# MuLabPKU/HD-PiSSA

Hardware: AMD Instinct MI355X
Metric: train tokens/sec (node) on the HD-PiSSA hot path, llama2-7b r16 (adapter probe fwd/bwd + Adam + dW aggregate + merge); dW merge+gather ms/step (higher is better)
Workload: dtype f32; 1 GPU; llama2-7b; model=llama2-7b, global_batch=16, seq_len=512, padding=per micro-batch to its longest sample (hp:190-201), micro_batches_per_rank=8, r_per_gpu=16, modules=224, exchange=gather, parallelism=dp1 (HD-PiSSA slices), x_layout=shared per projection group (q/k/v, gate/up)

## Files before the change

### hd-pissa_amd/csrc/hdp_probe.hip

```cpp
#include <chrono>
#include <cstdlib>
#include <cstring>
#include <mutex>
#include <vector>

#include "hdp_probe_int.h"

namespace hdp {

constexpr int kMaxGroup = 1024;
constexpr int kMaxSplit = 16;
constexpr int kP1Waves = 8;

static int p1_cols() {
  static const int v = [] { const char* e = getenv("HDP_P1_COLS"); return e ? atoi(e) : 128; }();
  return v;
}
static int p1_u() {
  static const int v = [] { const char* e = getenv("HDP_P1_U"); return e ? atoi(e) : 1; }();
  return v;
}
constexpr int kTC = 128;
constexpr int kNW = 256;

// ... 414 lines not shown
        const int j = 16 * b + 4 * g + reg;
        if (j >= r) continue;
        float* p = d.g + (int64_t)j * N + col;
        const f32x4 v{sc * acc2[b][0][reg], sc * acc2[b][1][reg], sc * acc2[b][2][reg], sc * acc2[b][3][reg]};
        if (vec) {
          gst4(p, d.acc ? gld4(p) + v : v);
        } else {
#pragma unroll
          for (int q = 0; q < 4; ++q)
            if (col + q < N) gst1(p + q, d.acc ? gld1(p + q) + v[q] : v[q]);
        }
      }
  } else {
    const bool v4 = (d.ldb & 3) == 0 && (reinterpret_cast<uintptr_t>(d.g) & 15) == 0;
#pragma unroll
    for (int b = 0; b < RB; ++b)
#pragma unroll
      for (int q = 0; q < 4; ++q) {
        if (col + q >= N) continue;
        const int j0 = 16 * b + 4 * g;
        float* p = d.g + (col + q) * d.ldb + j0;
        const f32x4 v = sc * acc2[b][q];
        if (v4 && j0 + 3 < r) {
          gst4(p, d.acc ? gld4(p) + v : v);
        } else {
#pragma unroll
          for (int reg = 0; reg < 4; ++reg)
            if (j0 + reg < r) gst1(p + reg, d.acc ? gld1(p + reg) + v[reg] : v[reg]);
        }
      }
  }
}

__device__ __forceinline__ void sw_store_g_fuse(const SweepDesc& d, const f32x4 (&acc2)[kSwMaxBlk][4], int64_t col,
                                                int g, bool vec) {
#pragma clang fp contract(off)
  const int64_t N = d.N;
  if (!d.part_t) {
#pragma unroll
    for (int b = 0; b < kSwMaxBlk; ++b) {
      if (b >= d.nb) break;
      const float sc = d.sc[b];
      const int acc = d.accb[b];
#pragma unroll
      for (int reg = 0; reg < 4; ++reg) {
        const int j = 4 * g + reg;
        if (j >= d.rbr[b]) continue;
        float* p = d.gb[b] + (int64_t)j * N + col;
        const f32x4 v{sc * acc2[b][0][reg], sc * acc2[b][1][reg], sc * acc2[b][2][reg], sc * acc2[b][3][reg]};
        if (vec) {
          gst4(p, acc ? gld4(p) + v : v);
        } else {
#pragma unroll
          for (int q = 0; q < 4; ++q)
            if (col + q < N) gst1(p + q, acc ? gld1(p + q) + v[q] : v[q]);
        }
      }
    }
  } else {
    const float sc = d.scale;
    const int r = d.r;
    const bool v4 = (d.ldb & 3) == 0 && (reinterpret_cast<uintptr_t>(d.g) & 15) == 0;
#pragma unroll
    for (int b = 0; b < kSwMaxBlk; ++b) {
      if (b >= d.nb) break;
#pragma unroll
      for (int q = 0; q < 4; ++q) {
        if (col + q >= N) continue;
        const int j0 = 16 * b + 4 * g;
        float* p = d.g + (col + q) * d.ldb + j0;
        const f32x4 v = sc * acc2[b][q];
        if (v4 && j0 + 3 < r) {
          gst4(p, d.acc ? gld4(p) + v : v);
        } else {
#pragma unroll
          for (int reg = 0; reg < 4; ++reg)
            if (j0 + reg < r) gst1(p + reg, d.acc ? gld1(p + reg) + v[reg] : v[reg]);
        }
      }
    }
  }
}

struct SweepArgs {
  int n, G;
  int spin;
  int64_t U;
  int* err;
  int* errd;
  const SweepDesc* d;
  const int* wst;
  const int* bnd;
};

template <int DT, int RB, int MODE, bool VEC, int OCC, bool FUSE, bool K32>
__device__ __forceinline__ void sweep_segment(const SweepDesc& d, int ct, int s0, int n, int64_t i0, int piece,
                                              const SweepArgs& sa, float* tile, float* red, int* flags, int wave,
                                              int lane) {
  constexpr bool PROJ = (MODE & kSwProj) != 0, OUTER = (MODE & kSwOuter) != 0;
  constexpr int rp = 16 * RB, r4 = rp / 4, ES = DT == HDP_F32 ? 4 : 2;
  const int li = lane & 15, g = lane >> 4;
  const int64_t T = d.T, N = d.N;
  const int64_t c = (int64_t)ct * kSwC + 64 * wave;
  const int64_t col = c + 4 * li;
  const int64_t colc = VEC ? (col < N ? col : N - 4) : col;
  const char* Zb = reinterpret_cast<const char*>(d.Z);

  constexpr bool SPLIT_F = DT == HDP_BF16 && MODE == kSwProj;
  constexpr bool X6 = K32 && DT == HDP_F32;
  constexpr bool K32P = K32 && MODE == kSwProj, K32O = K32 && MODE == kSwOuter;
  constexpr bool DL = K32P && DT == HDP_BF16 && !X6 && VEC;
  const int64_t cdl0 = c + 8 * g < N ? c + 8 * g : N - 8, cdl1 = c + 32 + 8 * g < N ? c + 32 + 8 * g : N - 8;
  f32x4 f[K32P ? 1 : 4][RB];
  bf16x4 fs[K32P ? 1 : 4][RB][3];
  bf16x8 fs8[K32P ? 2 : 1][RB][3];
  if constexpr (K32P) {
#pragma unroll
    for (int ch = 0; ch < 2; ++ch)
#pragma unroll
      for (int b = 0; b < RB; ++b) {
        const int j = 16 * b + li;
        const int64_t k = c + 32 * ch + 8 * g;
        float v[8];
#pragma unroll
        for (int e = 0; e < 8; ++e) v[e] = 0.f;
        const float* Fp = nullptr;
        int rows = d.r;
        if constexpr (FUSE) {
          Fp = b < d.nb ? d.Fb[b] : nullptr;
          rows = b < d.nb ? d.rbr[b] : 0;
        }
        const bool ok = FUSE ? (Fp != nullptr && li < rows) : (j < d.r);
        if (ok) {
          if (FUSE) Fp += (int64_t)li * N;
          if ((FUSE || d.f_rk) && N % 4 == 0 && k + 7 < N) {
            const float* P = FUSE ? Fp : d.F + (int64_t)j * N;
            const f32x4 a = gld4(P + k), bq = gld4(P + k + 4);
#pragma unroll
            for (int e = 0; e < 4; ++e) {
              v[e] = a[e];
              v[4 + e] = bq[e];
            }
          } else {
#pragma unroll
            for (int e = 0; e < 8; ++e)
              if (k + e < N)
                v[e] = FUSE ? gld1(Fp + k + e)
                            : d.f_rk ? gld1(d.F + (int64_t)j * N + k + e) : gld1(d.F + (k + e) * d.r + j);
          }
        }
        split8(v, fs8[ch][b][0], fs8[ch][b][1], fs8[ch][b][2]);
#pragma unroll
        for (int t = 0; t < 3; ++t) asm volatile("" : "+v"(fs8[ch][b][t]));
      }
  }
  if constexpr (PROJ && !K32P) {
#pragma unroll
    for (int s = 0; s < 4; ++s)
#pragma unroll
      for (int b = 0; b < RB; ++b) {
        const int j = 16 * b + li;
        const int64_t k = c + 16 * s + 4 * g;
        f32x4 v{0.f, 0.f, 0.f, 0.f};
        if constexpr (FUSE) {
          if (b < d.nb && li < d.rbr[b]) {
            const float* Fp = d.Fb[b] + (int64_t)li * N;
// ... 414 lines not shown
        load(z0, y0);
        if (k + 1 < nfull) compute(z1, y1, s0 + k + 1, i0 + k + 1, false);
      }
    }
  }
  if (nfull < n) {
    const int s = s0 + nfull;
    f32x4 z[4];
    float y[4][RB];
    if constexpr (DL) {
      typedef uint32_t u32x4d __attribute__((ext_vector_type(4)));
      int64_t row = 16 * (int64_t)s + li;
      row = row < T ? row : T - 1;
      z[0] = __builtin_bit_cast(f32x4, *reinterpret_cast<const HDP_GLOBAL u32x4d*>(gptr(Zb + (row * N + cdl0) * ES)));
      z[1] = __builtin_bit_cast(f32x4, *reinterpret_cast<const HDP_GLOBAL u32x4d*>(gptr(Zb + (row * N + cdl1) * ES)));
    }
#pragma unroll
    for (int p = 0; p < (DL ? 0 : 4); ++p) {
      int64_t row = 16 * (int64_t)s + 4 * p + g;
      row = row < T ? row : T - 1;
      if constexpr (VEC) {
        z[p] = load4<DT>(d.Z, row * N + colc);
      } else {
#pragma unroll
        for (int q = 0; q < 4; ++q) z[p][q] = load1<DT>(d.Z, row * N + (col + q < N ? col + q : N - 1));
      }
      if constexpr (OUTER) {
#pragma unroll
        for (int b = 0; b < RB; ++b) y[p][b] = gld1(d.y_in + row * d.yrs + li * d.yls + b);
      }
    }
    if constexpr (K32O)
      pair(z, y, z, y, s, false, true);
    else
      compute(z, y, s, i0 + nfull, true);
  }
  if constexpr (DIST) {
    if (pend_i >= 0) reduce_slice(pend_i, pend_s, pend_tail);
  }
  if constexpr (OUTER) {
    HDP_MFMA_FENCE();
    if (s0 == 0 && n == d.S) {
      if constexpr (FUSE) {
        if (col < N) sw_store_g_fuse(d, acc2, col, g, VEC);
      } else {
        if (col < N) sw_store_g<RB>(d, acc2, col, g, VEC);
      }
    } else if (FUSE && col < N) {
      const int64_t pofs = ((int64_t)ct * d.kmax + piece) * d.rpm * kSwC;
#pragma unroll
      for (int b = 0; b < RB; ++b) {
        if (b >= d.nb) break;
        float* base = d.part_b[b] + pofs;
        if (!d.part_t) {
#pragma unroll
          for (int reg = 0; reg < 4; ++reg)
            gst4(base + (4 * g + reg) * kSwC + 64 * wave + 4 * li,
                 f32x4{acc2[b][0][reg], acc2[b][1][reg], acc2[b][2][reg], acc2[b][3][reg]});
        } else {
#pragma unroll
          for (int q = 0; q < 4; ++q) gst4(base + (64 * wave + 4 * li + q) * d.rpm + 4 * g, acc2[b][q]);
        }
      }
    } else if (col < N) {
      float* base = d.part + ((int64_t)ct * d.kmax + piece) * rp * kSwC;
      if (!d.part_t) {
#pragma unroll
        for (int b = 0; b < RB; ++b)
#pragma unroll
          for (int reg = 0; reg < 4; ++reg)
            gst4(base + (16 * b + 4 * g + reg) * kSwC + 64 * wave + 4 * li,
                 f32x4{acc2[b][0][reg], acc2[b][1][reg], acc2[b][2][reg], acc2[b][3][reg]});
      } else {
#pragma unroll
        for (int b = 0; b < RB; ++b)
#pragma unroll
          for (int q = 0; q < 4; ++q)
            gst4(base + (64 * wave + 4 * li + q) * rp + 16 * b + 4 * g, acc2[b][q]);
      }
    }
  }
}

template <int DT, int RB, int MODE, bool VEC, int OCC, bool FUSE = false, bool K32 = false>
__global__ __launch_bounds__(512, OCC == 2 ? 4 : 2) void probe_sweep_kernel(SweepArgs sa) {
  extern __shared__ __attribute__((aligned(16))) float lds[];
  const int w = blockIdx.x;
  const int64_t nsteps = sa.bnd[w + 1] - sa.bnd[w];
  if (nsteps <= 0) return;
  const int lane = threadIdx.x & 63, wave = threadIdx.x >> 6;
  float* tile = lds + wave * 16 * kTileLd;
  float* red = lds + kSwWaves * 16 * kTileLd;
  int* flags = reinterpret_cast<int*>(red + sw_nbuf<RB, FUSE>() * kSwWaves * 16 * 16 * RB);
  if constexpr ((MODE & kSwProj) != 0) {
    if (threadIdx.x < 2 * sw_nbuf<RB, FUSE>()) flags[threadIdx.x] = 0;
    __syncthreads();
  }
  int m = sa.wst[4 * w], ct = sa.wst[4 * w + 1], s = sa.wst[4 * w + 2];
  int piece = sa.wst[4 * w + 3];
  for (int64_t done = 0; done < nsteps;) {
    const SweepDesc d = sa.d[m];
    const int n = (int)min((int64_t)(d.S - s), nsteps - done);
    sweep_segment<DT, RB, MODE, VEC, OCC, FUSE, K32>(d, ct, s, n, done, piece, sa, tile, red, flags, wave, lane);
    done += n;
    s = 0;
    piece = 0;
    if (++ct == d.nct) {
      ct = 0;
      ++m;
    }
  }
}

struct YReduceArgs {
  int n, rp;
  const YRedDesc* d;
};

__global__ __launch_bounds__(256) void probe_yreduce_kernel(YReduceArgs ya) {
  const YRedDesc d = ya.d[blockIdx.y];
  const int64_t f = (int64_t)blockIdx.x * 256 + threadIdx.x;
  const int64_t step4 = d.T * ya.rp / 4;
  if (f >= step4) return;
  const f32x4* src = reinterpret_cast<const f32x4*>(d.slab) + f;
  f32x4 acc{0.f, 0.f, 0.f, 0.f};
  for (int c0 = 0; c0 < d.nct; c0 += 8) {
    f32x4 v[8];
#pragma unroll
    for (int u = 0; u < 8; ++u) v[u] = c0 + u < d.nct ? gld4(reinterpret_cast<const float*>(src + (c0 + u) * step4)) : f32x4{0.f, 0.f, 0.f, 0.f};
#pragma unroll
    for (int u = 0; u < 8; ++u) acc += v[u];
  }
  const int rp = ya.rp;
  const int64_t e = 4 * f, t = e / rp;
  const int j0 = (int)(e % rp), b = j0 / 16, li0 = j0 % 16;
  float* dst = d.y + t * d.ys + b;
#pragma unroll
  for (int k = 0; k < 4; ++k) gst1(dst + (li0 + k) * d.sl, acc[k]);
}

struct SwFinishArgs {
  int n, rp;
  const FinDesc* d;
  const int* jobs;
  int bx;
};

template <int V>
__global__ __launch_bounds__(256) void probe_sweep_finish_kernel(SwFinishArgs fa) {
#pragma clang fp contract(off)
  typedef float vec __attribute__((ext_vector_type(V)));
  const int job = blockIdx.x / fa.bx;
  const FinDesc& dm = fa.d[fa.jobs[4 * job]];
  const int code = fa.jobs[4 * job + 1], ct = code >> 1;
  const bool sideA = (code & 1) == 0;
  const int r = dm.r;
  const int e = ((int)(blockIdx.x % fa.bx) * 256 + (int)threadIdx.x) * V;
  if (e >= r * kSwC) return;
  int nn, j;
  if (sideA) {
    j = e / kSwC;
    nn = e % kSwC;
  } else {
    nn = e / r;
    j = e % r;
  }
  const int64_t n = (int64_t)ct * kSwC + nn;
  if (n >= (sideA ? dm.in : dm.out)) return;
  const SwFinishSide& sd = sideA ? dm.sx : dm.sg;
  const int np = fa.jobs[4 * job + 2];
  const float* p = sd.part + (int64_t)ct * sd.kmax * fa.rp * kSwC + (sideA ? (int64_t)j * kSwC + nn : (int64_t)nn * fa.rp + j);
  const int64_t stride = (int64_t)fa.rp * kSwC;
  vec s0 = 0.f, s1 = 0.f;
  int k = 0;
  for (; k + 2 <= np; k += 2) {
    s0 += *reinterpret_cast<const HDP_GLOBAL vec*>(gptr(p + k * stride));
    s1 += *reinterpret_cast<const HDP_GLOBAL vec*>(gptr(p + (k + 1) * stride));
  }
  if (k < np) s0 += *reinterpret_cast<const HDP_GLOBAL vec*>(gptr(p + k * stride));
// ... 128 lines not shown
}

struct GroupWork {
  double xg = 0, fac = 0, x = 0, g = 0, s1 = 0, s2 = 0, fl_x = 0, fl_g = 0, fl_s1 = 0, fl_s2 = 0, grads = 0;
};
template <class GA>
static GroupWork group_work(const GA& ga, int es) {
  GroupWork w;
  for (int i = 0; i < ga.n; ++i) {
    const ProbeDesc& d = ga.d[i];
    const double X = (double)es * d.T * d.in, G = (double)es * d.T * d.out;
    const double fx = 2.0 * d.T * d.r * d.in, fg = 2.0 * d.T * d.r * d.out;
    w.x += X;
    w.g += G;
    w.fac += 4.0 * d.r * (d.in + d.out);
    w.fl_x += fx;
    w.fl_g += fg;
    const bool s1x = d.in <= d.out;
    w.s1 += s1x ? X : G;
    w.s2 += s1x ? G : X;
    w.fl_s1 += s1x ? fx : fg;
    w.fl_s2 += s1x ? fg : fx;
    w.grads += 4.0 * d.r * (d.in + d.out) * (d.accumulate ? 2 : 1);
  }
  w.xg = w.x + w.g;
  return w;
}

template <int DT, int RB>
static int launch_group(const GroupArgs& ga, hipStream_t st) {
  const GroupWork w = group_work(ga, DT == HDP_F32 ? 4 : 2);
  const int rp = ga.rp;
  const dim3 g1(ga.p1_pre[ga.n]), b1(kP1Waves * 64);
  auto lds1 = [&](int U) { return (size_t)kP1Waves * (16 * rp + U * 16 * kTileLd) * sizeof(float); };
  {
  KTimer kt(K_PROBE_P1, st, w.xg + w.fac, w.fl_x + w.fl_g);
  if constexpr (RB >= 4) {
    hipLaunchKernelGGL((probe_proj_kernel<DT, RB, 1>), g1, b1, lds1(1), st, ga);
  } else if constexpr (RB == 2) {
    hipLaunchKernelGGL((probe_proj_kernel<DT, RB, 1>), g1, b1, lds1(1), st, ga);
  } else {
    switch (p1_u()) {
      case 1: hipLaunchKernelGGL((probe_proj_kernel<DT, RB, 1>), g1, b1, lds1(1), st, ga); break;
      case 3: hipLaunchKernelGGL((probe_proj_kernel<DT, RB, 3>), g1, b1, lds1(3), st, ga); break;
      default: hipLaunchKernelGGL((probe_proj_kernel<DT, RB, 2>), g1, b1, lds1(2), st, ga); break;
    }
  }
  }
  HDP_CHECK_LAUNCH();
  {
    KTimer kt(K_PROBE_P2, st, w.xg, w.fl_x + w.fl_g);
    hipLaunchKernelGGL((probe_outer_kernel<DT, RB>), dim3(ga.p2_pre[ga.n]), dim3(512),
                       (size_t)(kTC * rp > 4096 ? kTC * rp : 4096) * sizeof(float), st, ga);
  }
  HDP_CHECK_LAUNCH();
  const int64_t tot = ga.p3_pre[ga.n];
  const int blocks = (int)min((int64_t)4096, (tot + 255) / 256);
  bool v4 = true;
  int64_t per = 1;
  for (int i = 0; i < ga.n; ++i) {
    const ProbeDesc& d = ga.d[i];
    v4 = v4 && d.r % 4 == 0 && d.in % 4 == 0 && (reinterpret_cast<uintptr_t>(d.gA) & 15) == 0 &&
         (reinterpret_cast<uintptr_t>(d.gB) & 15) == 0 && (reinterpret_cast<uintptr_t>(d.partA) & 15) == 0 &&
         (reinterpret_cast<uintptr_t>(d.partB) & 15) == 0;
    const int64_t e = ((int64_t)d.r * (d.in + d.out) + 1023) / 1024;
    per = e > per ? e : per;
  }
  {
    KTimer kt(K_PROBE_FINISH, st, w.grads);
    if (v4 && per < 65536)
      hipLaunchKernelGGL(probe_finish4_kernel, dim3((unsigned)per, (unsigned)ga.n), dim3(256), 0, st, ga);
    else
      hipLaunchKernelGGL(probe_finish_kernel, dim3(blocks), dim3(256), 0, st, ga);
  }
  HDP_CHECK_LAUNCH();
  return HDP_OK;
}

struct SweepKernel {
  void (*fn)(SweepArgs);
  size_t lds;
};

static SweepKnobs sweep_knobs() {
  auto on = [](const char* name) {
    const char* e = getenv(name);
    return !(e && e[0] == '0');
  };
  SweepKnobs kn;
  kn.share_x = on("HDP_PROBE_SHARE_X");
  kn.balance = on("HDP_PROBE_BALANCE");
  const char* e = getenv("HDP_PROBE_K32");
  kn.k32 = !e ? 2 : e[0] == '0' ? 0 : e[0] == '4' ? 1 : e[0] == 'a' ? 3 : 2;
  kn.x6 = on("HDP_PROBE_X6");
  return kn;
}

template <int DT, int RB, bool VEC>
static void pick_sweep(bool fuse, const SweepKnobs& kn, SweepKernel (&pk)[3]) {
  constexpr int rp = 16 * RB;
  constexpr bool BF = DT == HDP_BF16;
  constexpr bool SPLIT_B = RB >= 4 && BF;
  constexpr size_t proj_lds =
      ((size_t)kSwWaves * 16 * kTileLd + (size_t)sw_nbuf<RB>() * kSwWaves * 16 * rp) * sizeof(float) +
      2 * sw_nbuf<RB>() * 4;
  constexpr size_t fuse_lds =
      ((size_t)kSwWaves * 16 * kTileLd + (size_t)sw_nbuf<kSwMaxBlk, true>() * kSwWaves * 16 * 16 * kSwMaxBlk) *
          sizeof(float) +
      2 * sw_nbuf<kSwMaxBlk, true>() * 4;
  constexpr int OCC_B = SPLIT_B ? 1 : RB >= 4 ? 3 : VEC ? 2 : 1;
  constexpr int MODE_B = SPLIT_B ? kSwProj : kSwProj | kSwOuter;
  constexpr bool CAN_FUSE = RB <= 2;
  constexpr int RBF = CAN_FUSE ? kSwMaxBlk : RB;
  const int k32m = BF ? kn.k32 : 0;
  const bool k32 = k32m >= 2 || (k32m == 1 && RB >= 4);
  const bool k32c = k32m == 3 || (k32m >= 1 && RB >= 4);
  const bool x6 = !BF && fuse && kn.x6;
  const bool kf = k32 || x6;
  const bool fused = CAN_FUSE && fuse;
  constexpr bool K32B = BF && MODE_B == kSwProj;
  if (fused) {
    if constexpr (CAN_FUSE)
      pk[0] = {kf ? probe_sweep_kernel<DT, RBF, kSwProj, VEC, 1, true, true>
                  : probe_sweep_kernel<DT, RBF, kSwProj, VEC, 1, true>,
               fuse_lds};
  } else {
    pk[0] = {k32 ? probe_sweep_kernel<DT, RB, kSwProj, VEC, 1, false, BF> : probe_sweep_kernel<DT, RB, kSwProj, VEC, 1>,
             proj_lds};
  }
  pk[1] = {k32 ? probe_sweep_kernel<DT, RB, MODE_B, VEC, OCC_B, false, K32B>
               : probe_sweep_kernel<DT, RB, MODE_B, VEC, OCC_B>,
           proj_lds};
  if (fused) {
    if constexpr (CAN_FUSE)
      pk[2] = {k32 ? probe_sweep_kernel<DT, RBF, kSwOuter, VEC, 1, true, BF>
                   : probe_sweep_kernel<DT, RBF, kSwOuter, VEC, 1, true>,
               0};
  } else {
    pk[2] = {k32c ? probe_sweep_kernel<DT, RB, kSwOuter, VEC, 1, false, BF> : probe_sweep_kernel<DT, RB, kSwOuter, VEC, 1>,
             0};
  }
}

static int sweep_slots(const SweepKernel& k) {
  struct Entry {
    void (*fn)(SweepArgs);
    int dev, slots;
  };
  static std::mutex mu;
  static std::vector<Entry> cache;
  int dev = 0;
  if (hipGetDevice(&dev) != hipSuccess || dev < 0) dev = 0;
  std::lock_guard<std::mutex> lk(mu);
  for (const Entry& e : cache)
    if (e.fn == k.fn && e.dev == dev) return e.slots;
  int cus = 0, per = 0;
  if (hipDeviceGetAttribute(&cus, hipDeviceAttributeMultiprocessorCount, dev) != hipSuccess || cus <= 0) cus = 256;
  if (hipOccupancyMaxActiveBlocksPerMultiprocessor(&per, k.fn, 512, k.lds) != hipSuccess || per <= 0) per = 1;
  cache.push_back(Entry{k.fn, dev, cus * per});
  return cus * per;
}

template <int DT, int RB, bool VEC>
static int launch_sweep(const HostGroup& ga, char* tab, hipStream_t st) {
  constexpr int rp = 16 * RB;
  const int n = ga.n;
  const SweepKnobs kn = sweep_knobs();
  SweepSides s;
  plan_sweep_sides(ga, DT == HDP_BF16, kn, s);
  SweepKernel pk[3];
  pick_sweep<DT, RB, VEC>(s.fuse, kn, pk);
  const int slots[3] = {sweep_slots(pk[0]), sweep_slots(pk[1]), sweep_slots(pk[2])};
  SweepTables t;
  const SweepError pe = plan_sweep_tables(ga, s, slots, t);
  static_assert(kSweepEInval == HDP_EINVAL, "the planner's error code");
  if (pe.code != 0) {
    set_error("%s", pe.msg);
    return pe.code;
  }
  const int rc = probe_tables_upload(t.blob, tab, st);
  if (rc) return rc;

  int* err = probe_err_word();
  HDP_CHECK_ARG(err != nullptr, "probe sweep: error word allocation failed");
  int* errd = probe_err_local();
  const int spin = probe_spin();
  static const int kid[3] = {K_SWEEP_A, K_SWEEP_B, K_SWEEP_C};
  auto sweep = [&](int ph) {
    const SweepArgs sa{(int)s.sd[ph].size(), t.G[ph], spin, s.U[ph], err, errd,
                       reinterpret_cast<const SweepDesc*>(tab + t.o_sd[ph]), reinterpret_cast<const int*>(tab + t.o_w[ph]),
                       reinterpret_cast<const int*>(tab + t.o_b[ph])};
    KTimer kt(kid[ph], st, s.bytes_ph[ph], s.flop_ph[ph]);
    hipLaunchKernelGGL(pk[ph].fn, dim3(t.G[ph]), dim3(512), pk[ph].lds, st, sa);
  };
  auto reduce = [&](int k) {
    KTimer kt(K_PROBE_REDUCE, st, s.slab[k]);
    hipLaunchKernelGGL(probe_yreduce_kernel, dim3((unsigned)s.yblk, (unsigned)n), dim3(256), 0, st,
                       YReduceArgs{n, rp, reinterpret_cast<const YRedDesc*>(tab + t.o_y[k])});
  };
  sweep(0);
  HDP_CHECK_LAUNCH();
  reduce(0);
  HDP_CHECK_LAUNCH();
  sweep(1);
  HDP_CHECK_LAUNCH();
  reduce(1);
  HDP_CHECK_LAUNCH();
  sweep(2);
  HDP_CHECK_LAUNCH();
  if (t.njobs) {
    const int V = s.v4 ? 4 : 1;
    const int bx = (rp * kSwC + 256 * V - 1) / (256 * V);
    SwFinishArgs fa{n, rp, reinterpret_cast<const FinDesc*>(tab + t.o_f), reinterpret_cast<const int*>(tab + t.o_j), bx};
    KTimer kt(K_PROBE_FINISH, st, t.pieces);
    if (s.v4)
      hipLaunchKernelGGL(probe_sweep_finish_kernel<4>, dim3((unsigned)(t.njobs * bx)), dim3(256), 0, st, fa);
    else
      hipLaunchKernelGGL(probe_sweep_finish_kernel<1>, dim3((unsigned)(t.njobs * bx)), dim3(256), 0, st, fa);
    HDP_CHECK_LAUNCH();
  }
  return HDP_OK;
}

}

using namespace hdp;

static size_t module_bytes(int64_t T, int64_t in, int64_t out, int r) {
  size_t b = plan_module(T, in, out, r).bytes;
  if (r > 64 && r <= 128 && use_sweep(4)) {
    size_t sl = 0;
    const int ns = n_slices(r);
    for (int k = 0; k < ns; ++k) sl += plan_module(T, in, out, (r + ns - 1) / ns).bytes;
    b = sl > b ? sl : b;
  }
  return b;
}

extern "C" size_t hdp_probe_workspace_bytes(int64_t T, int64_t in, int64_t out, int r) {
  if (T <= 0 || in <= 0 || out <= 0 || r <= 0 || r > 128) return 0;
  return module_bytes(T, in, out, r);
}

extern "C" int hdp_probe_group_max(void) { return kMaxGroup; }

extern "C" int hdp_probe_errors(int clear) { return probe_err_read(clear); }

extern "C" int64_t hdp_probe_host_wait_us(int reset) {
  std::lock_guard<std::mutex> lk(g_stage_mu);
  const int64_t us = g_wait_ns / 1000;
// ... 336 lines not shown
```

Baseline: 194,400 tokens/s.

## Add software-pipelined seam sweep kernel with prefetched Z/Y loads across segments

Adds a new sweep path for f32 vector-load kernels that runs a worker's whole step range as one flat loop. It keeps a two- or three-deep ring of prefetched Z/Y register buffers that crosses segment and module boundaries, loads descriptors through constant address space, and batches old-gradient loads ahead of stores at segment seams. The aim is to hide global load latency and per-segment restart overhead in the probe projection/outer-product sweeps. The cost is much higher register pressure and a large amount of new, complex code. It is on by default for f32, disabled through HDP_PROBE_SEAM=0, and is only used when the problem dimensions fit in 32-bit offsets.

Result: no change. 197,700 tokens/s (median of 2 runs) (+1.7%).

```diff
diff --git a/hd-pissa_amd/csrc/hdp_probe.hip b/hd-pissa_amd/csrc/hdp_probe.hip
--- a/hd-pissa_amd/csrc/hdp_probe.hip
+++ b/hd-pissa_amd/csrc/hdp_probe.hip
@@ -520,6 +520,83 @@
   }
 }
 
+template <int RB, bool FUSE>
+__device__ __forceinline__ void sw_store_g_seam(const SweepDesc& d, const f32x4 (&acc2)[RB][4], int64_t col, int g) {
+#pragma clang fp contract(off)
+  const int64_t N = d.N;
+  const int nb = FUSE ? d.nb : RB;
+  f32x4 old[RB][4];
+  auto landed = [&]() {
+#pragma unroll
+    for (int b = 0; b < RB; ++b)
+#pragma unroll
+      for (int k = 0; k < 4; ++k) asm volatile("" : "+v"(old[b][k]));
+  };
+  if (!d.part_t) {
+    auto row = [&](int b, int reg, float*& p, bool& acc) {
+      const int j = 4 * g + reg;
+      acc = FUSE ? d.accb[b] != 0 : d.acc != 0;
+      p = (FUSE ? d.gb[b] + (int64_t)j * N : d.g + (int64_t)(16 * b + j) * N) + col;
+      return FUSE ? j < d.rbr[b] : 16 * b + j < d.r;
+    };
+#pragma unroll
+    for (int b = 0; b < RB; ++b) {
+      if (b >= nb) break;
+#pragma unroll
+      for (int reg = 0; reg < 4; ++reg) {
+        float* p;
+        bool acc;
+        if (row(b, reg, p, acc) && acc) old[b][reg] = gld4(p);
+      }
+    }
+    landed();
+#pragma unroll
+    for (int b = 0; b < RB; ++b) {
+      if (b >= nb) break;
+      const float sc = FUSE ? d.sc[b] : d.scale;
+#pragma unroll
+      for (int reg = 0; reg < 4; ++reg) {
+        float* p;
+        bool acc;
+        if (!row(b, reg, p, acc)) continue;
+        const f32x4 v{sc * acc2[b][0][reg], sc * acc2[b][1][reg], sc * acc2[b][2][reg], sc * acc2[b][3][reg]};
+        gst4(p, acc ? old[b][reg] + v : v);
+      }
+    }
+  } else {
+    const float sc = d.scale;
+    const int r = d.r;
+    const bool acc = d.acc != 0;
+    const bool v4 = (d.ldb & 3) == 0 && (reinterpret_cast<uintptr_t>(d.g) & 15) == 0;
+#pragma unroll
+    for (int b = 0; b < RB; ++b) {
+      if (b >= nb) break;
+#pragma unroll
+      for (int q = 0; q < 4; ++q)
+        if (col + q < N && v4 && 16 * b + 4 * g + 3 < r && acc) old[b][q] = gld4(d.g + (col + q) * d.ldb + 16 * b + 4 * g);
+    }
+    landed();
+#pragma unroll
+    for (int b = 0; b < RB; ++b) {
+      if (b >= nb) break;
+#pragma unroll
+      for (int q = 0; q < 4; ++q) {
+        if (col + q >= N) continue;
+        const int j0 = 16 * b + 4 * g;
+        float* p = d.g + (col + q) * d.ldb + j0;
+        const f32x4 v = sc * acc2[b][q];
+        if (v4 && j0 + 3 < r) {
+          gst4(p, acc ? old[b][q] + v : v);
+        } else {
+#pragma unroll
+          for (int reg = 0; reg < 4; ++reg)
+            if (j0 + reg < r) gst1(p + reg, acc ? gld1(p + reg) + v[reg] : v[reg]);
+        }
+      }
+    }
+  }
+}
+
 struct SweepArgs {
   int n, G;
   int spin;
@@ -1100,7 +1177,385 @@
   }
 }
 
-template <int DT, int RB, int MODE, bool VEC, int OCC, bool FUSE = false, bool K32 = false>
+template <int RB, int MODE, int OCC, bool FUSE>
+__device__ __forceinline__ void sweep_range_seam(const SweepArgs& sa, int w, int64_t nsteps, float* tile, float* red,
+                                                 int* flags, int wave, int lane) {
+  constexpr bool PROJ = (MODE & kSwProj) != 0, OUTER = (MODE & kSwOuter) != 0;
+  constexpr int rp = 16 * RB, r4 = rp / 4;
+  static_assert(!(PROJ && !FUSE && RB >= 4), "SEAM: no distributed hand-off");
+  static_assert(OCC == 1 || OCC == 2, "SEAM: three or two register sets");
+  const int li = lane & 15, g = lane >> 4;
+  wave = __builtin_amdgcn_readfirstlane(wave);
+
+  int m = sa.wst[4 * w], ct = sa.wst[4 * w + 1], s = sa.wst[4 * w + 2];
+  int piece = sa.wst[4 * w + 3];
+  const __attribute__((address_space(4))) SweepDesc* dtab =
+      (const __attribute__((address_space(4))) SweepDesc*)sa.d;
+  SweepDesc d;
+  auto fetch_desc = [&](SweepDesc& to, int mi) {
+    typedef uint32_t u32x4k __attribute__((ext_vector_type(4)));
+    static_assert(sizeof(SweepDesc) % 16 == 0, "SweepDesc copied in 16-byte words");
+    const __attribute__((address_space(4))) u32x4k* src = (const __attribute__((address_space(4))) u32x4k*)(dtab + mi);
+    u32x4k* dst = reinterpret_cast<u32x4k*>(&to);
+#pragma unroll
+    for (int k = 0; k < (int)(sizeof(SweepDesc) / 16); ++k) dst[k] = src[k];
+  };
+  fetch_desc(d, m);
+  int left = (int)nsteps;
+  int i = 0;
+  int seg_left = min(d.S - s, left);
+  bool whole = s == 0 && seg_left == d.S;
+  int64_t T = d.T, N = d.N;
+  int c = ct * kSwC + 64 * wave;
+
+  f32x4 f[4][RB];
+  auto load_frags = [&](int li, int g) {
+    if constexpr (PROJ) {
+#pragma unroll
+      for (int ss = 0; ss < 4; ++ss)
+#pragma unroll
+        for (int b = 0; b < RB; ++b) {
+          const int j = 16 * b + li;
+          const int64_t k = c + 16 * ss + 4 * g;
+          f32x4 v{0.f, 0.f, 0.f, 0.f};
+          if constexpr (FUSE) {
+            if (b < d.nb && li < d.rbr[b]) {
+              const float* Fp = d.Fb[b] + (int64_t)li * N;
+              if (N % 4 == 0 && k + 3 < N) {
+                v = gld4(Fp + k);
+              } else {
+#pragma unroll
+                for (int q = 0; q < 4; ++q)
+                  if (k + q < N) v[q] = gld1(Fp + k + q);
+              }
+            }
+          } else if (j < d.r) {
+            if (d.f_rk && N % 4 == 0 && k + 3 < N) {
+              v = gld4(d.F + (int64_t)j * N + k);
+            } else {
+#pragma unroll
+              for (int q = 0; q < 4; ++q)
+                if (k + q < N) v[q] = d.f_rk ? gld1(d.F + (int64_t)j * N + k + q) : gld1(d.F + (k + q) * d.r + j);
+            }
+          }
+          f[ss][b] = v;
+        }
+#pragma unroll
+      for (int ss = 0; ss < 4; ++ss)
+#pragma unroll
+        for (int b = 0; b < RB; ++b) asm volatile("" : "+v"(f[ss][b]));
+    }
+  };
+
+  bool hs_broken = false;
+  f32x4 acc2[OUTER ? RB : 1][4];
+  auto zero_acc = [&]() {
+#pragma unroll
+    for (int b = 0; b < (OUTER ? RB : 1); ++b)
+#pragma unroll
+      for (int q = 0; q < 4; ++q) acc2[b][q] = f32x4{0.f, 0.f, 0.f, 0.f};
+  };
+  zero_acc();
+
+  auto compute = [&](const f32x4 (&z)[4], const float (&y)[4][RB], bool tail) {
+    const int rows = (int)T - 16 * s;
+    if constexpr (OUTER) {
+#pragma unroll
+      for (int p = 0; p < 4; ++p) {
+#pragma unroll
+        for (int b = 0; b < RB; ++b) {
+          if (FUSE && b >= d.nb) break;
+          const float yv = y[p][b];
+#pragma unroll
+          for (int q = 0; q < 4; ++q) acc2[b][q] = __builtin_amdgcn_mfma_f32_16x16x4f32(yv, z[p][q], acc2[b][q], 0, 0, 0);
+        }
+      }
+    }
+    if constexpr (PROJ) {
+#pragma unroll
+      for (int p = 0; p < 4; ++p) *reinterpret_cast<f32x4*>(tile + (4 * p + g) * kTileLd + 4 * li) = z[p];
+      f32x4 a0[RB], a1[RB];
+#pragma unroll
+      for (int b = 0; b < RB; ++b) a0[b] = a1[b] = f32x4{0.f, 0.f, 0.f, 0.f};
+#pragma unroll
+      for (int ss = 0; ss < 4; ++ss) {
+        const f32x4 zf = *reinterpret_cast<const f32x4*>(tile + li * kTileLd + 16 * ss + 4 * g);
+#pragma unroll
+        for (int b = 0; b < RB; ++b) {
+          if (FUSE && b >= d.nb) break;
+#pragma unroll
+          for (int q = 0; q < 4; ++q) {
+            if (ss & 1) a1[b] = __builtin_amdgcn_mfma_f32_16x16x4f32(zf[q], f[ss][b][q], a1[b], 0, 0, 0);
+            else a0[b] = __builtin_amdgcn_mfma_f32_16x16x4f32(zf[q], f[ss][b][q], a0[b], 0, 0, 0);
+          }
+        }
+      }
+      HDP_MFMA_FENCE();
+      constexpr int NBUF = sw_nbuf<RB, FUSE>();
+      int iw = i;
+      asm volatile("" : "+s"(iw));
+      const int bsel = iw % NBUF;
+      const int round = iw / NBUF;
+      int* arrive = flags + bsel;
+      int* done = flags + NBUF + bsel;
+      if (round > 0 && !hs_broken) {
+        int it = 0;
+        while (sa.spin < 0 || __hip_atomic_load(done, __ATOMIC_RELAXED, __HIP_MEMORY_SCOPE_WORKGROUP) < round) {
+          if (it++ >= sa.spin) {
+            hs_broken = true;
+            if (lane == 0) {
+              __hip_atomic_store(sa.err, 1, __ATOMIC_RELAXED, __HIP_MEMORY_SCOPE_SYSTEM);
+              __hip_atomic_store(sa.errd, 1, __ATOMIC_RELAXED, __HIP_MEMORY_SCOPE_AGENT);
+            }
+            break;
+          }
+          __builtin_amdgcn_s_sleep(1);
+        }
+        asm volatile("" ::: "memory");
+      }
+      float* rb = red + (bsel * kSwWaves + wave) * 16 * rp;
+#pragma unroll
+      for (int b = 0; b < RB; ++b) {
+        if (FUSE && b >= d.nb) break;
+#pragma unroll
+        for (int reg = 0; reg < 4; ++reg) rb[(4 * g + reg) * rp + 16 * b + li] = a0[b][reg] + a1[b][reg];
+      }
+      asm volatile("s_waitcnt lgkmcnt(0)" ::: "memory");
+      int old = 0;
+      if (lane == 0) old = __hip_atomic_fetch_add(arrive, 1, __ATOMIC_RELAXED, __HIP_MEMORY_SCOPE_WORKGROUP);
+      old = __builtin_amdgcn_readfirstlane(old);
+      if (old == kSwWaves - 1) {
+        asm volatile("s_waitcnt lgkmcnt(0)" ::: "memory");
+        const float* rs = red + bsel * kSwWaves * 16 * rp;
+        int ln = lane;
+        asm volatile("" : "+v"(ln));
+        if constexpr (FUSE) {
+#pragma unroll
+          for (int b = 0; b < RB; ++b) {
+            if (b >= d.nb) break;
+            const int row = ln >> 2, jj = (ln & 3) * 4;
+            f32x4 acc{0.f, 0.f, 0.f, 0.f};
+#pragma unroll
+            for (int ww = 0; ww < kSwWaves; ++ww)
+              acc += *reinterpret_cast<const f32x4*>(rs + (ww * 16 + row) * rp + 16 * b + jj);
+            const int64_t t = 16 * (int64_t)s + row;
+            if (!tail || row < rows) gst4(d.slab_b[b] + ((int64_t)ct * T + t) * d.rpm + jj, acc);
+          }
+        } else {
+#pragma unroll
+          for (int e0 = 0; e0 < 16 * r4; e0 += 64) {
+            const int e = e0 + ln, row = e / r4, j = (e % r4) * 4;
+            f32x4 acc{0.f, 0.f, 0.f, 0.f};
+#pragma unroll
+            for (int ww = 0; ww < kSwWaves; ++ww) acc += *reinterpret_cast<const f32x4*>(rs + (ww * 16 + row) * rp + j);
+            const int64_t t = 16 * (int64_t)s + row;
+            if (!tail || row < rows) gst4(d.slab_out + ((int64_t)ct * T + t) * rp + j, acc);
+          }
+        }
+        asm volatile("s_waitcnt lgkmcnt(0)" ::: "memory");
+        if (lane == 0) {
+          __hip_atomic_store(arrive, 0, __ATOMIC_RELAXED, __HIP_MEMORY_SCOPE_WORKGROUP);
+          __hip_atomic_store(done, round + 1, __ATOMIC_RELAXED, __HIP_MEMORY_SCOPE_WORKGROUP);
+        }
+      }
+    }
+  };
+
+  auto seam = [&]() {
+    int ln = lane;
+    asm volatile("" : "+v"(ln));
+    const int li = ln & 15, g = ln >> 4;
+    const int64_t col = (int64_t)c + 4 * li;
+    if constexpr (OUTER) {
+      int mf = m;
+      asm volatile("" : "+s"(mf));
+      SweepDesc d;
+      fetch_desc(d, mf);
+      HDP_MFMA_FENCE();
+      if (whole) {
+        if constexpr (FUSE) {
+          if (col < N) sw_store_g_seam<RB, FUSE>(d, acc2, col, g);
+        } else {
+          if (col < N) sw_store_g<RB>(d, acc2, col, g, true);
+        }
+      } else if (FUSE && col < N) {
+        const int64_t pofs = ((int64_t)ct * d.kmax + piece) * d.rpm * kSwC;
+#pragma unroll
+        for (int b = 0; b < RB; ++b) {
+          if (b >= d.nb) break;
+          float* base = d.part_b[b] + pofs;
+          if (!d.part_t) {
+#pragma unroll
+            for (int reg = 0; reg < 4; ++reg)
+              gst4(base + (4 * g + reg) * kSwC + 64 * wave + 4 * li,
+                   f32x4{acc2[b][0][reg], acc2[b][1][reg], acc2[b][2][reg], acc2[b][3][reg]});
+          } else {
+#pragma unroll
+            for (int q = 0; q < 4; ++q) gst4(base + (64 * wave + 4 * li + q) * d.rpm + 4 * g, acc2[b][q]);
+          }
+        }
+      } else if (col < N) {
+        float* base = d.part + ((int64_t)ct * d.kmax + piece) * rp * kSwC;
+        if (!d.part_t) {
+#pragma unroll
+          for (int b = 0; b < RB; ++b)
+#pragma unroll
+            for (int reg = 0; reg < 4; ++reg)
+              gst4(base + (16 * b + 4 * g + reg) * kSwC + 64 * wave + 4 * li,
+                   f32x4{acc2[b][0][reg], acc2[b][1][reg], acc2[b][2][reg], acc2[b][3][reg]});
+        } else {
+#pragma unroll
+          for (int b = 0; b < RB; ++b)
+#pragma unroll
+            for (int q = 0; q < 4; ++q)
+              gst4(base + (64 * wave + 4 * li + q) * rp + 16 * b + 4 * g, acc2[b][q]);
+        }
+      }
+      zero_acc();
+    }
+    if (left > 0) {
+      s = 0;
+      piece = 0;
+      if (++ct == d.nct) {
+        ct = 0;
+        ++m;
+        fetch_desc(d, m);
+        T = d.T;
+        N = d.N;
+      }
+      seg_left = min(d.S, left);
+      whole = seg_left == d.S;
+      c = ct * kSwC + 64 * wave;
+      if constexpr (PROJ) load_frags(li, g);
+    }
+  };
+
+  int lm = m, lct = ct, ls = s;
+  int lrem = (int)nsteps;
+  const char* LZ = reinterpret_cast<const char*>(d.Z);
+  const float* LY = d.y_in;
+  int LN = (int)d.N, LT = (int)d.T;
+  int Lyrs = d.yrs, Lyls = d.yls, LS = d.S, Lnct = d.nct;
+  auto lane_col = [&]() {
+    const int lcol = lct * kSwC + 64 * wave + 4 * li;
+    return lcol < LN ? lcol : LN - 4;
+  };
+  int lcolc = lane_col();
+  uint32_t zoff0 = (uint32_t)(g * LN + lcolc) * 4u, yoff0 = (uint32_t)(g * Lyrs + li * Lyls) * 4u;
+  auto load = [&](f32x4 (&z)[4], float (&y)[4][RB]) {
+    __builtin_amdgcn_sched_barrier(0);
+    const int rmax = LT - 1 - 16 * ls;
+    const char* zb = LZ + (int64_t)(16 * ls) * LN * 4;
+    const char* yb = reinterpret_cast<const char*>(LY + (int64_t)(16 * ls) * Lyrs);
+    auto issue = [&](int p, const char* zp, const char* yp8) {
+      z[p] = __builtin_nontemporal_load(reinterpret_cast<const HDP_GLOBAL f32x4*>(gptr(zp)));
+      if constexpr (OUTER) {
+        const float* yp = reinterpret_cast<const float*>(yp8);
+        if constexpr (RB == 4) {
+          const f32x4 v = gld4(yp);
+#pragma unroll
+          for (int b = 0; b < RB; ++b) y[p][b] = v[b];
+        } else {
+#pragma unroll
+          for (int b = 0; b < RB; ++b) y[p][b] = gld1(yp + b);
+        }
+      }
+    };
+    const char *zbp[4], *ybp[4];
+    uint32_t zo[4], yo[4];
+    if (rmax >= 15) {
+#pragma unroll
+      for (int p = 0; p < 4; ++p) {
+        zbp[p] = zb + (int64_t)(4 * p) * LN * 4;
+        ybp[p] = yb + (int64_t)(4 * p) * Lyrs * 4;
+        zo[p] = zoff0;
+        yo[p] = yoff0;
+      }
+    } else {
+#pragma unroll
+      for (int p = 0; p < 4; ++p) {
+        int rr = 4 * p + g;
+        rr = rr < rmax ? rr : rmax;
+        zbp[p] = zb;
+        ybp[p] = yb;
+        zo[p] = (uint32_t)(rr * LN + lcolc) * 4u;
+        yo[p] = (uint32_t)(rr * Lyrs + li * Lyls) * 4u;
+      }
+    }
+#pragma unroll
+    for (int p = 0; p < 4; ++p) issue(p, zbp[p] + zo[p], ybp[p] + yo[p]);
+    __builtin_amdgcn_sched_barrier(0);
+    --lrem;
+    if (++ls == LS) {
+      ls = 0;
+      if (++lct == Lnct) {
+        lct = 0;
+        ++lm;
+        if (lrem > 0) {
+          const __attribute__((address_space(4))) SweepDesc& dn = dtab[lm];
+          LZ = reinterpret_cast<const char*>(dn.Z);
+          LY = dn.y_in;
+          LN = (int)dn.N;
+          LT = (int)dn.T;
+          Lyrs = dn.yrs;
+          Lyls = dn.yls;
+          LS = dn.S;
+          Lnct = dn.nct;
+        }
+      }
+      lcolc = lane_col();
+      zoff0 = (uint32_t)(g * LN + lcolc) * 4u;
+      yoff0 = (uint32_t)(g * Lyrs + li * Lyls) * 4u;
+    }
+  };
+  auto step = [&](const f32x4 (&z)[4], float (&y)[4][RB]) {
+    const bool tail = 16 * ((int64_t)s + 1) > T;
+    if constexpr (OUTER) {
+      if (tail) {
+        const int rows = (int)T - 16 * s;
+#pragma unroll
+        for (int p = 0; p < 4; ++p)
+#pragma unroll
+          for (int b = 0; b < RB; ++b) y[p][b] = 4 * p + g < rows ? y[p][b] : 0.f;
+      }
+    }
+    compute(z, y, tail);
+    ++s;
+    ++i;
+    --left;
+    if (--seg_left == 0) seam();
+  };
+
+  if constexpr (PROJ) load_frags(li, g);
+  constexpr int NS = OCC == 1 ? 3 : 2;
+  f32x4 zz[NS][4];
+  float yy[NS][4][RB];
+  if (lrem >= 2 * NS - 1) {
+#pragma unroll
+    for (int j = 0; j + 1 < NS; ++j) load(zz[j], yy[j]);
+    while (lrem >= NS) {
+#pragma unroll
+      for (int j = 0; j < NS; ++j) {
+        load(zz[(j + NS - 1) % NS], yy[(j + NS - 1) % NS]);
+        step(zz[j], yy[j]);
+      }
+    }
+  } else {
+#pragma unroll
+    for (int j = 0; j + 1 < NS; ++j)
+      if (lrem > 0) load(zz[j], yy[j]);
+  }
+#pragma unroll
+  for (int j = 0; j < NS; ++j) {
+    if (lrem > 0) load(zz[(j + NS - 1) % NS], yy[(j + NS - 1) % NS]);
+    if (left > 0) step(zz[j], yy[j]);
+  }
+#pragma unroll
+  for (int j = 0; j + 2 < NS; ++j)
+    if (left > 0) step(zz[j], yy[j]);
+}
+
+template <int DT, int RB, int MODE, bool VEC, int OCC, bool FUSE = false, bool K32 = false, bool SEAM = false>
 __global__ __launch_bounds__(512, OCC == 2 ? 4 : 2) void probe_sweep_kernel(SweepArgs sa) {
   extern __shared__ __attribute__((aligned(16))) float lds[];
   const int w = blockIdx.x;
@@ -1113,6 +1568,11 @@
   if constexpr ((MODE & kSwProj) != 0) {
     if (threadIdx.x < 2 * sw_nbuf<RB, FUSE>()) flags[threadIdx.x] = 0;
     __syncthreads();
+  }
+  if constexpr (SEAM) {
+    static_assert(DT == HDP_F32 && VEC && !K32, "SEAM instances: float32 MFMA forms, vector loads");
+    sweep_range_seam<RB, MODE, OCC, FUSE>(sa, w, nsteps, tile, red, flags, wave, lane);
+    return;
   }
   int m = sa.wst[4 * w], ct = sa.wst[4 * w + 1], s = sa.wst[4 * w + 2];
   int piece = sa.wst[4 * w + 3];
@@ -1407,22 +1867,27 @@
   size_t lds;
 };
 
-static SweepKnobs sweep_knobs() {
+struct SweepLaunchKnobs : SweepKnobs {
+  bool seam = true;
+};
+
+static SweepLaunchKnobs sweep_knobs() {
   auto on = [](const char* name) {
     const char* e = getenv(name);
     return !(e && e[0] == '0');
   };
-  SweepKnobs kn;
+  SweepLaunchKnobs kn;
   kn.share_x = on("HDP_PROBE_SHARE_X");
   kn.balance = on("HDP_PROBE_BALANCE");
   const char* e = getenv("HDP_PROBE_K32");
   kn.k32 = !e ? 2 : e[0] == '0' ? 0 : e[0] == '4' ? 1 : e[0] == 'a' ? 3 : 2;
   kn.x6 = on("HDP_PROBE_X6");
+  kn.seam = on("HDP_PROBE_SEAM");
   return kn;
 }
 
 template <int DT, int RB, bool VEC>
-static void pick_sweep(bool fuse, const SweepKnobs& kn, SweepKernel (&pk)[3]) {
+static void pick_sweep(bool fuse, const SweepLaunchKnobs& kn, SweepKernel (&pk)[3]) {
   constexpr int rp = 16 * RB;
   constexpr bool BF = DT == HDP_BF16;
   constexpr bool SPLIT_B = RB >= 4 && BF;
@@ -1444,6 +1909,8 @@
   const bool kf = k32 || x6;
   const bool fused = CAN_FUSE && fuse;
   constexpr bool K32B = BF && MODE_B == kSwProj;
+  constexpr bool CAN_SEAM = !BF && VEC;
+  const bool seam = CAN_SEAM && kn.seam;
   if (fused) {
     if constexpr (CAN_FUSE)
       pk[0] = {kf ? probe_sweep_kernel<DT, RBF, kSwProj, VEC, 1, true, true>
@@ -1456,11 +1923,15 @@
   pk[1] = {k32 ? probe_sweep_kernel<DT, RB, MODE_B, VEC, OCC_B, false, K32B>
                : probe_sweep_kernel<DT, RB, MODE_B, VEC, OCC_B>,
            proj_lds};
+  if constexpr (CAN_SEAM && RB == 1)
+    if (seam) pk[1].fn = probe_sweep_kernel<DT, RB, MODE_B, VEC, OCC_B, false, false, true>;
   if (fused) {
     if constexpr (CAN_FUSE)
       pk[2] = {k32 ? probe_sweep_kernel<DT, RBF, kSwOuter, VEC, 1, true, BF>
                    : probe_sweep_kernel<DT, RBF, kSwOuter, VEC, 1, true>,
                0};
+    if constexpr (CAN_FUSE && CAN_SEAM)
+      if (seam) pk[2].fn = probe_sweep_kernel<DT, RBF, kSwOuter, VEC, 1, true, false, true>;
   } else {
     pk[2] = {k32c ? probe_sweep_kernel<DT, RB, kSwOuter, VEC, 1, false, BF> : probe_sweep_kernel<DT, RB, kSwOuter, VEC, 1>,
              0};
@@ -1490,7 +1961,9 @@
 static int launch_sweep(const HostGroup& ga, char* tab, hipStream_t st) {
   constexpr int rp = 16 * RB;
   const int n = ga.n;
-  const SweepKnobs kn = sweep_knobs();
+  SweepLaunchKnobs kn = sweep_knobs();
+  for (int i = 0; i < n; ++i)
+    kn.seam = kn.seam && ga.d[i].in < (1 << 26) && ga.d[i].out < (1 << 26) && ga.d[i].T < (1ll << 31) - 16;
   SweepSides s;
   plan_sweep_sides(ga, DT == HDP_BF16, kn, s);
   SweepKernel pk[3];
```
